# agordon/fastx_toolkit

Measured on AMD Instinct MI355X. Metric: Mreads/s (150 bp) quality-trim+filter, higher is better.
Workload: dtype u8

## Files before the change

fastx_toolkit_amd/csrc/fxg_kernels.h:

```cpp
#pragma once
#include "fxg_device.h"
#include "fxg_clip_instances.h"

#define FXG_INVALID_TUPLE 0xFFFFFFFFu

#define FXG_NTALLY 16
struct FxgLds {
    u32 slot_bytes, so_ksrc, so_kidx, so_ktab;
    u32 off_scratch, off_tally, off_bm_g, off_bm_l, off_bases, off_ptab, total;
    u32 has_tab;
};
__host__ __device__ inline u32 fxg_r16(u32 x) { return (x + 15u) & ~15u; }
__host__ __device__ inline FxgLds fxg_lds_layout(u32 T, u32 stride, u32 bitmaps, u32 stage_stride, u32 nslots = 2, bool no_tab = false, u32 ptab_bytes = 0u)
{
    FxgLds l;
    l.so_ksrc = fxg_r16((T + 1) * 4);
    l.so_kidx = l.so_ksrc + fxg_r16(T * 4);
    l.so_ktab = l.so_kidx + fxg_r16(T * 2);
    l.has_tab = (stage_stride || no_tab) ? 0u : 1u;
    l.slot_bytes = l.so_ktab + (l.has_tab ? fxg_r16(((T * stride + 15) / 16 + 1) * 2) : 0u);
    u32 o = nslots * l.slot_bytes;
    l.off_scratch = o; o += fxg_r16(48 * 4);
    l.off_tally = o;   o += FXG_NTALLY * 8;
    const u32 words = (T * stride + 31) / 32 + 2;
    l.off_bm_g = o;    o += bitmaps ? fxg_r16(words * 4) * (bitmaps == 4u ? 4u : 1u) : 0;
    l.off_bm_l = bitmaps == 1u ? l.off_bm_g : o;    o += bitmaps == 2u ? fxg_r16(words * 4) : 0;
    l.off_bases = o;   o += stage_stride ? fxg_r16(T * stage_stride + 16) : 0;
    l.off_ptab = o;    o += fxg_r16(ptab_bytes);
    l.total = o;
    return l;
}

FXG_HD u32 fxg_bitmap_count(const FxgKArgs &a, bool use_q, bool clip) { return !use_q ? 0u : (clip && a.tq == a.fq) ? 1u : 2u; }

#ifdef FXG_HOST_EMULATION
FXG_HD int fxg_wave_max(int n) { return n; }
#else
__device__ __forceinline__ int fxg_wave_max(int n)
{
    int v = n;
#pragma unroll
    for (int d = 1; d < 64; d <<= 1) { const int o = __shfl_xor(v, d, 64); v = o > v ? o : v; }
    return __builtin_amdgcn_readfirstlane(v);
}
#endif

FXG_HD void fxg_clip_finish(const FxgKArgs &a, int len, int qs, int ts, int mism, int sz, int matches, int bq, int first_n,
                            u32 *out_len, u32 *keep, u32 *reason, u32 *clipped, u32 *adapter_only)
{
    int i = -1;
    if (sz != 0 && !(a.clip_min_adapter_len > 0 && sz < a.clip_min_adapter_len)) {
        if (bq == len - 1 && mism == 0) i = qs;
        else if (sz > 5 && ts == 0 && matches * 100 >= 75 * sz) i = qs;
        else if (sz > 11 && matches * 100 >= 80 * sz) i = qs;
        else if (len >= 2 && bq >= len - 2 && sz <= 5 && matches >= 3) i = qs;
    }
    int cur = len;
    u32 k = 1, why = FXG_R_KEPT, cl = 0, ao = 0;
    if (i > 0) { i += a.clip_keep_delta; if (i < cur) cur = i; cl = 1; }
    if (i == 0) {
        ao = 1;
        if (!(a.clip_flags & FXG_CLIP_ADAPTER_ONLY)) { k = 0; why = FXG_R_CLIP_ADAPTER_ONLY; }
    } else if ((u32)cur < a.clip_min_len) { k = 0; why = FXG_R_CLIP_TOO_SHORT; }
    else if (i == -1 && (a.clip_flags & FXG_CLIP_DISCARD_NON_CLIPPED)) { k = 0; why = FXG_R_CLIP_NO_ADAPTER; }
    else if (i > 0 && (a.clip_flags & FXG_CLIP_DISCARD_CLIPPED)) { k = 0; why = FXG_R_CLIP_ADAPTER_FOUND; }
    else if (!(a.clip_flags & FXG_CLIP_KEEP_N) && first_n < cur) { k = 0; why = FXG_R_CLIP_N; }
    else if (a.clip_flags & FXG_CLIP_ADAPTER_ONLY) { k = 0; why = FXG_R_CLIP_K_MODE; }
    *out_len = (u32)cur; *keep = k; *reason = why; *clipped = cl; *adapter_only = ao;
}

template <int AMAX>
FXG_HD void fxg_clip_read(const FxgKArgs &a, const uint8_t *rd, int len, int rows,
                          u32 *out_len, u32 *keep, u32 *reason, u32 *clipped, u32 *adapter_only, const bool UR = false)
{
    float S[AMAX];
    u32 W0[AMAX], W1[AMAX];
    const int A = a.alen;
#pragma unroll
    for (int t = 0; t < AMAX; ++t) {
        S[t] = (t <= 3) ? 0.0f : -5.0f * (float)(t - 3);
        W0[t] = FXG_INVALID_TUPLE; W1[t] = 0u;
    }
    float best = -1000000.0f;
    u32 bw0 = FXG_INVALID_TUPLE, bw1 = 0u, bq = 0u;
    int first_n = len;
    const int rows_u = UR ? rows : fxg_wave_max(rows);
#pragma unroll 1
    for (int q = 0; q < rows_u; ++q) {
        if (q >= rows) continue;
        const u32 c = rd[q];
        const bool qn = (c == (u32)'N');
        first_n = (qn && first_n == len && q < len) ? q : first_n;
        float dS = 0.0f, uS = 0.0f;
        u32 dW0 = FXG_INVALID_TUPLE, dW1 = 0u, uW0 = FXG_INVALID_TUPLE, uW1 = 0u;
#pragma unroll
        for (int t = 0; t < AMAX; ++t) {
            const u32 tc = (u32)(uint8_t)a.adapter[t];
            const bool tn = (tc == (u32)'N');
            const bool eq = (c == tc);
            const bool neutral = qn || tn;
            const float pair = neutral ? ((qn && tn) ? 0.0f : 0.1f) : (eq ? 1.0f : -1.0f);
            const float ul = dS + pair;
            const float up = uS + -5.0f;
            float left = S[t] + -5.0f;
            if (t > 3) left = (t - 3 > q) ? -100000.0f : left;
            const bool g1 = up > ul;
            float sc = g1 ? up : ul;
            u32 w0 = g1 ? uW0 : dW0, w1 = g1 ? uW1 : dW1;
            const bool g2 = left > sc;
            sc = g2 ? left : sc;
            w0 = g2 ? W0[t] : w0; w1 = g2 ? W1[t] : w1;
            const bool diag = !(g1 || g2);
            const bool fresh = (w0 == FXG_INVALID_TUPLE);
            w0 = fresh ? (((u32)q << 16) | ((u32)t << 8)) : w0;
            w1 = fresh ? 0u : w1;
            w1 += 0x10000u + ((diag && !neutral && eq) ? 1u : 0u);
            w0 += (diag && !neutral && !eq) ? 1u : 0u;
            dS = S[t]; dW0 = W0[t]; dW1 = W1[t];
            S[t] = sc; W0[t] = w0; W1[t] = w1;
            uS = sc; uW0 = w0; uW1 = w1;
            const bool gb = (sc > best) && (t < A);
            best = gb ? sc : best; bw0 = gb ? w0 : bw0; bw1 = gb ? w1 : bw1; bq = gb ? (u32)q : bq;
        }
    }
    fxg_clip_finish(a, len, (int)(bw0 >> 16), (int)((bw0 >> 8) & 0xFFu), (int)(bw0 & 0xFFu), (int)(bw1 >> 16), (int)(bw1 & 0xFFFFu),
                    (int)bq, first_n, out_len, keep, reason, clipped, adapter_only);
}

#define FXG_PK_MAT1  1u
#define FXG_PK_SZ1   (1u << 5)
#define FXG_PK_DIA1  (1u << 14)

template <int AMAX> struct FxgClip2 {
    static constexpr int SPAN = AMAX + (AMAX + 1) / 5;
    static constexpr int C = SPAN / 2 > 0 ? SPAN / 2 : 1;
    static constexpr int WIN = 3 * C;
};

#define FXG_PTAB_LUT_BYTES 512u
#define FXG_PTAB_ROW_BYTES 64u
__host__ __device__ constexpr bool fxg_clip_uses_ptab(int amax) { return amax < 0; }
FXG_HD u32 fxg_ptab_rows(const char *adapter, int alen)
{
    u32 r = 2u;
    for (int t = 0; t < alen; ++t) {
        bool seen = adapter[t] == 'N';
        for (int u = 0; u < t; ++u) seen = seen || (adapter[u] == adapter[t]);
        r += seen ? 0u : 1u;
    }
    return r;
}
FXG_HD u32 fxg_ptab_stride(u32 cols) { const u32 s = (cols * 4u + 15u) & ~15u; return cols <= 16u ? FXG_PTAB_ROW_BYTES : (((s >> 4) & 1u) ? s : s + 16u); }
FXG_HD u32 fxg_ptab_bytes(u32 rows, u32 stride) { return FXG_PTAB_LUT_BYTES + 2u * rows * stride; }
#define FXG_PTAB_MAX_ROWS_K 8u

FXG_HD void fxg_ptab_row_map(const char *adapter, int alen, uint8_t (&row)[256])
{
    for (int b = 0; b < 256; ++b) row[b] = 0u;
    row[0] = 0x80u;
    u32 next = 2u;
    for (int t = 0; t < alen; ++t) {
        const u32 c = (u32)(uint8_t)adapter[t];
        if (c == (u32)'N' || row[c] != 0u) continue;
        row[c] = (uint8_t)(0x80u | next++);
    }
    row[(u32)'N'] = 0x80u | 1u;
}

FXG_HD void fxg_clip_ptab_build(const FxgKArgs &a, uint8_t *ptab, u32 tid, u32 nthreads)
{
    uint16_t *lut = reinterpret_cast<uint16_t *>(ptab);
    const int COLS = (int)a.clip_ptab_cols, A = a.alen < COLS ? a.alen : COLS;
    const u32 R = a.clip_ptab_rows, ST = a.clip_ptab_stride;
    for (u32 b = tid; b < 256u; b += nthreads) {
        const u32 e = a.clip_ptab_row[b], row = e & 0x7Fu;
        lut[b] = (uint16_t)(FXG_PTAB_LUT_BYTES + row * ST);
        if (e & 0x80u) {
            float *pv = reinterpret_cast<float *>(ptab + FXG_PTAB_LUT_BYTES + row * ST);
            u32 *sv = reinterpret_cast<u32 *>(ptab + FXG_PTAB_LUT_BYTES + (R + row) * ST);
            for (int t = 0; t < COLS; ++t) {
                const u32 tc = t < A ? (u32)(uint8_t)a.adapter[t] : 0u;
                const bool eq = tc == b, qn = b == (u32)'N', tn = tc == (u32)'N';
                pv[t] = tn ? (qn ? 0.0f : 0.1f) : (qn ? 0.1f : (eq ? 1.0f : -1.0f));
                sv[t] = (tn || qn) ? 0u : a.clip_ptab_dia1 + (eq ? 1u : 0u);
            }
        }
    }
}

#ifndef FXG_HOST_EMULATION
#define FXG_SCHED_FENCE() __builtin_amdgcn_sched_barrier(0)
#else
#define FXG_SCHED_FENCE() ((void)0)
#endif

FXG_HD float fxg_minus5() { return -5.0f; }

template <int AMAX, bool STEPS>
FXG_HD void fxg_ptab_fetch(const uint8_t *ptab, u32 off, u32 step_off, u32 (&pr)[16], u32 (&st)[16])
{
    const u32x4 *p = reinterpret_cast<const u32x4 *>(ptab + off);
#pragma unroll
    for (int k = 0; k < (AMAX + 3) / 4; ++k) { const u32x4 v = p[k]; pr[4 * k] = v.x; pr[4 * k + 1] = v.y; pr[4 * k + 2] = v.z; pr[4 * k + 3] = v.w; }
    if constexpr (STEPS) {
        const u32x4 *g = reinterpret_cast<const u32x4 *>(ptab + off + step_off);
#pragma unroll
        for (int k = 0; k < (AMAX + 3) / 4; ++k) { const u32x4 v = g[k]; st[4 * k] = v.x; st[4 * k + 1] = v.y; st[4 * k + 2] = v.z; st[4 * k + 3] = v.w; }
    }
}

template <int AMAX, bool EARLY, bool STEPS = false>
FXG_HD float fxg_clip_row_score_t(int A, int q, float (&S)[AMAX], float (&Sm)[AMAX], u32 (&pr)[16], u32 (&st)[16], const uint8_t *ptab, u32 o_next, u32 step_off)
{
    constexpr int AMIN = AMAX <= 4 ? 1 : (AMAX <= 8 ? 5 : AMAX);
    float ul[AMAX];
#pragma unroll
    for (int t = 0; t < AMAX; ++t) ul[t] = (t ? S[t - 1] : 0.0f) + __builtin_bit_cast(float, pr[t]);
    FXG_SCHED_FENCE();
    fxg_ptab_fetch<AMAX, STEPS>(ptab, o_next, step_off, pr, st);
    FXG_SCHED_FENCE();
    const float m5 = fxg_minus5();
    float uSm = -5.0f, rowmax = -1000000.0f;
#pragma unroll
    for (int t = 0; t < AMAX; ++t) {
        float left = Sm[t];
        if (EARLY && t > 3) left = (t - 3 > q) ? -100000.0f : left;
        const float sc = fmaxf(fmaxf(ul[t], uSm), left);
        const float scm = sc + m5;
        S[t] = sc; Sm[t] = scm; uSm = scm;
        if (t < AMIN) rowmax = fmaxf(rowmax, sc);
        else rowmax = (t < A) ? fmaxf(rowmax, sc) : rowmax;
    }
    return rowmax;
}

template <int AMAX, bool EARLY, bool TRACK>
FXG_HD void fxg_clip_row_packed_t(int A, int q, u32 vstart, float (&S)[AMAX], float (&Sm)[AMAX], u32 (&W)[AMAX], float &best, u32 &bw, u32 &bq,
                                  u32 (&pr)[16], u32 (&st)[16], const uint8_t *ptab, u32 o_next, u32 step_off)
{
    const float best_in = best;
    float ul[AMAX];
    u32 wd[AMAX];
#pragma unroll
    for (int t = 0; t < AMAX; ++t) {
        ul[t] = (t ? S[t - 1] : 0.0f) + __builtin_bit_cast(float, pr[t]);
        wd[t] = (t ? W[t - 1] : 0u) + st[t];
    }
    FXG_SCHED_FENCE();
    fxg_ptab_fetch<AMAX, true>(ptab, o_next, step_off, pr, st);
    FXG_SCHED_FENCE();
    const float m5 = fxg_minus5();
    float uSm = -5.0f;
    u32 uW = 0u;
#pragma unroll
    for (int t = 0; t < AMAX; ++t) {
        const float up = uSm;
        float left = Sm[t];
        if (EARLY && t > 3) left = (t - 3 > q) ? -100000.0f : left;
        const float sc = fmaxf(fmaxf(ul[t], up), left);
        const bool isd = (sc == ul[t]), isu = (sc == up);
        u32 w;
        if (t == 0) {
            const u32 src = (isd || isu) ? 0u : W[0];
            const u32 step = isd ? wd[0] : 0u;
            w = (src == 0u) ? ((vstart << 24) + FXG_PK_SZ1 + step) : (src + step);
        } else {
            w = isu ? uW : W[t];
            w = isd ? wd[t] : w;
        }
        const u32 wp = w + FXG_PK_SZ1;
        const float scm = sc + m5;
        S[t] = sc; Sm[t] = scm; W[t] = wp;
        uSm = scm; uW = wp;
        constexpr int AMIN = AMAX <= 4 ? 1 : (AMAX <= 8 ? 5 : (AMAX <= 16 ? AMAX : AMAX - 3));
        if (!TRACK) continue;
        if (t < AMIN) {
            const bool gb = sc > best;
            bw = gb ? w : bw;
            best = fmaxf(best, sc);
        } else {
            const bool gb = (sc > best) && (t < A);
            best = gb ? sc : best; bw = gb ? w : bw;
        }
    }
    if (TRACK) bq = (best > best_in) ? (u32)q : bq;
}

FXG_HD int fxg_gl_last_dword(u64 total, u64 off)
{
    const u64 left = total > off ? (total - off) >> 2 : 0;
    return left == 0 ? 0 : (left - 1 > (u64)0x7FFFFFFF ? 0x7FFFFFFF : (int)(left - 1));
}

FXG_HD u32 fxg_ld32(const uint8_t *row, int i, int imax)
{
    const int k = i < imax ? i : imax;
#ifdef FXG_HOST_EMULATION
    u32 w; memcpy(&w, row + 4 * (size_t)k, 4); return w;
#else
    return reinterpret_cast<const u32 *>(row)[k];
#endif
}

FXG_HD int fxg_clip_first_n(const uint8_t *rd, int len, int len_u, u32 stride, int first_n)
{
    if ((stride & 3u) == 0u) {
#pragma unroll 1
        for (int k = (len_u + 3) / 4 - 1; k >= 0; --k) {
#ifdef FXG_HOST_EMULATION
            u32 w; memcpy(&w, rd + 4 * k, 4);
#else
            const u32 w = reinterpret_cast<const u32 *>(rd)[k];
#endif
            const u32 v = w ^ 0x4E4E4E4Eu;
            const u32 z = (v - 0x01010101u) & ~v & 0x80808080u;
            const int pos = 4 * k + (int)((u32)__builtin_ctz(z | 0x80000000u) >> 3);
            first_n = (z != 0u && pos < len) ? pos : first_n;
        }
    } else {
#pragma unroll 1
        for (int k = len_u - 1; k >= 0; --k) first_n = (k < len && rd[k] == (uint8_t)'N') ? k : first_n;
    }
    return first_n;
}

template <int AMAX, bool GL = false>
FXG_HD int fxg_clip_two_pass(const FxgKArgs &a, const uint8_t *rd, int len, int rows, float &best, u32 &bw, u32 &bq, int &first_n, const bool UR = false, const uint8_t *ptab = nullptr)
{
    constexpr int C = FxgClip2<AMAX>::C;
    float S[AMAX], Sm[AMAX], P0[AMAX], P1[AMAX], P2[AMAX], CB[AMAX];
    const int A = a.alen;
#pragma unroll
    for (int t = 0; t < AMAX; ++t) { S[t] = (t <= 3) ? 0.0f : -5.0f * (float)(t - 3); Sm[t] = S[t] + -5.0f; P0[t] = P1[t] = P2[t] = CB[t] = S[t]; }
    const int early_rows = (A - 4 < rows) ? (A - 4 > 0 ? A - 4 : 0) : rows;
    const int rows_u = UR ? rows : fxg_wave_max(rows > 0 ? rows : 0);
    if (rows_u <= 0) return 0;
    float b1 = -1000000.0f;
    int q = 0, r0 = 0, bq1 = 0;
    u32 cn = 0u, gw0 = 0u, gw1 = 0u;
    int gmax = 0;
    u32 pr[16] = {}, st[16] = {}, on = 0u;
    const u32 step_off = a.clip_ptab_rows * a.clip_ptab_stride;
    const uint16_t *lut = reinterpret_cast<const uint16_t *>(ptab);
    if constexpr (GL) {
        gmax = fxg_gl_last_dword(a.clip_total, (u64)(rd - a.clip_src));
        gw0 = fxg_ld32(rd, 0, gmax); gw1 = fxg_ld32(rd, 1, gmax);
        on = lut[(gw0 >> 8) & 0xFFu];
        fxg_ptab_fetch<AMAX, false>(ptab, lut[gw0 & 0xFFu], step_off, pr, st);
    } else {
        const u32 o0 = lut[rd[0]];
        on = lut[rd[1]]; cn = rd[2];
        fxg_ptab_fetch<AMAX, false>(ptab, o0, step_off, pr, st);
    }
#define FXG_CLIP_CHUNK(EARLY, Psave, Pwin)                                                                                   \
    {                                                                                                                        \
        _Pragma("unroll") for (int t = 0; t < AMAX; ++t) Psave[t] = S[t];                                                    \
        const int q0 = q, qend = q + C < rows_u ? q + C : rows_u;                                                            \
        bool upd = false;                                                                                                    \
        _Pragma("unroll 1") for (; q < qend; ++q) {                                                                          \
            float rm;                                                                                                        \
            if constexpr (GL) {                   \
                const u32 ca = ((((q + 2) >> 2) == (q >> 2) ? gw0 : gw1) >> ((u32)((q + 2) & 3) << 3)) & 0xFFu;             \
                const u32 on2 = lut[ca];                                                                                     \
                if ((q & 3) == 3) { gw0 = gw1; gw1 = fxg_ld32(rd, (q >> 2) + 2, gmax); }                                     \
                if (!UR && q >= rows) continue;                                                                              \
                rm = fxg_clip_row_score_t<AMAX, EARLY>(A, q, S, Sm, pr, st, ptab, on, step_off);                             \
                on = on2;                                                                                                    \
            } else {                                                                                                         \
                if (!UR && q >= rows) continue;           \
                const u32 on2 = lut[cn];                                                                                     \
                cn = rd[q + 3];                                                                                              \
                rm = fxg_clip_row_score_t<AMAX, EARLY>(A, q, S, Sm, pr, st, ptab, on, step_off);                             \
                on = on2;                                                                                                    \
            }                                                                                                                \
            const bool g = rm > b1;                                                                                          \
            b1 = g ? rm : b1; bq1 = g ? q : bq1; upd = upd || g;                                                             \
        }                                                                                                                    \
        if (upd) {                                                                                                           \
            _Pragma("unroll") for (int t = 0; t < AMAX; ++t) CB[t] = Pwin[t];                                                \
            r0 = q0 - 2 * C > 0 ? q0 - 2 * C : 0;                                                                            \
        }                                                                                                                    \
    }
    static_assert(2 * C >= AMAX - 4, "early rows must end inside the first two chunks");
    FXG_CLIP_CHUNK(true, P0, P1)
    if (q < rows_u) FXG_CLIP_CHUNK(true, P1, P2)
    while (q < rows_u) {
        FXG_CLIP_CHUNK(false, P2, P0)
        if (q >= rows_u) break;
        FXG_CLIP_CHUNK(false, P0, P1)
        if (q >= rows_u) break;
        FXG_CLIP_CHUNK(false, P1, P2)
    }
#undef FXG_CLIP_CHUNK
    if (rows <= 0) return 0;
    if (FXG_DBG(a, 32u)) { best = b1; bq = (u32)bq1; bw = 0u; return 0; }
    u32 W[AMAX];
#pragma unroll
    for (int t = 0; t < AMAX; ++t) { S[t] = CB[t]; Sm[t] = CB[t] + -5.0f; W[t] = ((u32)(t + 1) << 19) + FXG_PK_SZ1; }
    q = r0;
    constexpr int SPAN = FxgClip2<AMAX>::SPAN;
    const int rs = bq1 - SPAN + 1 > r0 ? bq1 - SPAN + 1 : r0;
    const int qlast = rows - 1;
#define FXG_RD_AHEAD(i) rd[GL && (i) > qlast ? qlast : (i)]
    {
        const u32 o0 = lut[rd[q]];
        on = lut[FXG_RD_AHEAD(q + 1)]; cn = FXG_RD_AHEAD(q + 2);
        fxg_ptab_fetch<AMAX, true>(ptab, o0, step_off, pr, st);
    }
    const int n0 = rs - r0, n0u = fxg_wave_max(n0);
#pragma unroll 1
    for (int i = 0; i < n0u; ++i) {
        if (i >= n0) continue;
        const u32 on2 = lut[cn];
        cn = FXG_RD_AHEAD(q + 3);
        (void)fxg_clip_row_score_t<AMAX, true, true>(A, q, S, Sm, pr, st, ptab, on, step_off);
        on = on2; ++q;
    }
    const int win = bq1 - rs, n1 = win < early_rows ? win : early_rows, n2 = win - n1;
    const int n1u = fxg_wave_max(n1), n2u = fxg_wave_max(n2);
#pragma unroll 1
    for (int i = 0; i < n1u; ++i) {
        if (i >= n1) continue;
        const u32 on2 = lut[cn];
        cn = FXG_RD_AHEAD(q + 3);
        fxg_clip_row_packed_t<AMAX, true, false>(A, q, (u32)(q - rs), S, Sm, W, best, bw, bq, pr, st, ptab, on, step_off);
        on = on2; ++q;
    }
#pragma unroll 1
    for (int i = 0; i < n2u; ++i) {
        if (i >= n2) continue;
        const u32 on2 = lut[cn];
        cn = FXG_RD_AHEAD(q + 3);
        fxg_clip_row_packed_t<AMAX, false, false>(A, q, (u32)(q - rs), S, Sm, W, best, bw, bq, pr, st, ptab, on, step_off);
        on = on2; ++q;
    }
    fxg_clip_row_packed_t<AMAX, true, true>(A, bq1, (u32)(bq1 - rs), S, Sm, W, best, bw, bq, pr, st, ptab, on, step_off);
#undef FXG_RD_AHEAD
    if (!(a.clip_flags & FXG_CLIP_KEEP_N)) first_n = fxg_clip_first_n(rd, len, UR ? len : fxg_wave_max(len), a.clip_stride, first_n);
    return rs;
}

#define FXG_K_MAT1 1u
#define FXG_K_DIA1 (1u << 7)
#define FXG_K_SZ1  (1u << 14)
#define FXG_K_START(v) ((u32)(v) << 23)
__host__ __device__ constexpr int fxg_clip_k_amin(int amax) { return amax <= 16 ? 1 : fxg_clip_bucket_below(amax) + 1; }
static_assert(fxg_clip_k_amin(16) == 1 && fxg_clip_k_amin(20) == 17 && fxg_clip_k_amin(24) == 21 && fxg_clip_k_amin(64) == 61 && fxg_clip_k_amin(72) == 65 &&
              fxg_clip_k_amin(88) == 81 && fxg_clip_k_amin(100) == 89, "a bucket's smallest adapter is the next smaller bucket + 1");
template <int AMAX> struct FxgClipK { static constexpr bool SM = AMAX <= 24; static constexpr int NSM = SM ? AMAX : 1; };

template <int AMAX, bool EARLY, bool TRACK>
FXG_HD void fxg_clip_row_kt(const FxgKArgs &a, int A, u32 c, int q, u32 vstart, float (&S)[AMAX], float (&Sm)[FxgClipK<AMAX>::NSM], u32 (&W)[AMAX],
                            float &best, u32 &bw, u32 &bq, const uint8_t *ptab)
{
    constexpr bool SM = FxgClipK<AMAX>::SM;
    constexpr int AMIN = fxg_clip_k_amin(AMAX);
    const u32 po = reinterpret_cast<const uint16_t *>(ptab)[c & 0xFFu];
    const u32x4 *pp = reinterpret_cast<const u32x4 *>(ptab + po), *sp = reinterpret_cast<const u32x4 *>(ptab + po + a.clip_ptab_rows * a.clip_ptab_stride);
    const float best_in = best, m5 = fxg_minus5();
    float uSm = -5.0f;
    u32 uW = 0u;
    u32x4 cp = pp[0], cs = sp[0];
    float ul = 0.0f + __builtin_bit_cast(float, cp.x);
    u32 wd = cs.x;
#pragma unroll
    for (int kb = 0; kb < AMAX; kb += 4) {
        u32x4 np = cp, ns = cs;
        if (kb + 4 < AMAX) { np = pp[kb / 4 + 1]; ns = sp[kb / 4 + 1]; }
#pragma unroll
        for (int j = 0; j < 4; ++j) {
            const int t = kb + j;
            if (t >= AMAX) break;
            float ul_next = 0.0f;
            u32 wd_next = 0u;
            if (t + 1 < AMAX) {
                const u32 pv = j == 0 ? cp.y : j == 1 ? cp.z : j == 2 ? cp.w : np.x;
                const u32 sv = j == 0 ? cs.y : j == 1 ? cs.z : j == 2 ? cs.w : ns.x;
                ul_next = S[t] + __builtin_bit_cast(float, pv);
                wd_next = W[t] + sv;
            }
            float left = SM ? Sm[SM ? t : 0] : S[t] + m5;
            if (EARLY && t > 3) left = (t - 3 > q) ? -100000.0f : left;
            const float sc = fmaxf(fmaxf(ul, uSm), left);
            const bool isd = (sc == ul), isu = (sc == uSm);
            u32 w;
            if (t == 0) {
                const u32 fresh = FXG_K_START(vstart) + FXG_K_SZ1 + (isd ? wd : 0u);
                w = (isd || isu) ? fresh : W[0];
            } else {
                w = isu ? uW : W[t];
                w = isd ? wd : w;
            }
            const u32 wp = w + FXG_K_SZ1;
            const float scm = sc + m5;
            S[t] = sc; W[t] = wp;
            if (SM) Sm[SM ? t : 0] = scm;
            uSm = scm; uW = wp; ul = ul_next; wd = wd_next;
            if (!TRACK) continue;
            if (t < AMIN) {
                const bool gb = sc > best;
                bw = gb ? w : bw;
                best = fmaxf(best, sc);
            } else {
                const bool gb = (sc > best) && (t < A);
                best = gb ? sc : best; bw = gb ? w : bw;
            }
        }
        cp = np; cs = ns;
    }
    if (TRACK) bq = (best > best_in) ? (u32)q : bq;
}

template <int AMAX, bool EARLY, bool TRACK>
FXG_HD void fxg_clip_row_k(const FxgKArgs &a, int A, u32 c, int q, u32 vstart, float (&S)[AMAX], float (&Sm)[FxgClipK<AMAX>::NSM], u32 (&W)[AMAX],
                           float &best, u32 &bw, u32 &bq, const uint8_t *ptab)
{
    fxg_clip_row_kt<AMAX, EARLY, TRACK>(a, A, c, q, vstart, S, Sm, W, best, bw, bq, ptab);
}

template <int AMAX, bool EARLY>
FXG_HD float fxg_clip_row_score_k(const FxgKArgs &a, int A, u32 c, int q, float (&S)[AMAX], float (&Sm)[AMAX], const uint8_t *ptab)
{
    constexpr bool SM = AMAX <= 48;
    constexpr int AMIN = fxg_clip_k_amin(AMAX);
    const u32 po = reinterpret_cast<const uint16_t *>(ptab)[c & 0xFFu];
    const u32x4 *pp = reinterpret_cast<const u32x4 *>(ptab + po);
    const float m5 = fxg_minus5();
    float uSm = -5.0f, rowmax = -1000000.0f;
    u32x4 cp = pp[0];
    float ul = 0.0f + __builtin_bit_cast(float, cp.x);
#pragma unroll
    for (int kb = 0; kb < AMAX; kb += 4) {
        u32x4 np = cp;
        if (kb + 4 < AMAX) np = pp[kb / 4 + 1];
#pragma unroll
        for (int j = 0; j < 4; ++j) {
            const int t = kb + j;
            if (t >= AMAX) break;
            float ul_next = 0.0f;
            if (t + 1 < AMAX) ul_next = S[t] + __builtin_bit_cast(float, j == 0 ? cp.y : j == 1 ? cp.z : j == 2 ? cp.w : np.x);
            float left = SM ? Sm[SM ? t : 0] : S[t] + m5;
            if (EARLY && t > 3) left = (t - 3 > q) ? -100000.0f : left;
            const float sc = fmaxf(fmaxf(ul, uSm), left);
            const float scm = sc + m5;
            S[t] = sc;
            if (SM) Sm[SM ? t : 0] = scm;
            uSm = scm; ul = ul_next;
            if (t < AMIN) rowmax = fmaxf(rowmax, sc);
            else rowmax = (t < A) ? fmaxf(rowmax, sc) : rowmax;
        }
        cp = np;
    }
    return rowmax;
}

template <int AMAX>
FXG_HD void fxg_clip_rows_k(const FxgKArgs &a, const uint8_t *rd, int len, int rows, float &best, u32 &bw, u32 &bq, int &first_n, const bool UR = false, const uint8_t *ptab = nullptr)
{
    float S[AMAX], Sm[FxgClipK<AMAX>::NSM];
    u32 W[AMAX];
    const int A = a.alen;
#pragma unroll
    for (int t = 0; t < AMAX; ++t) {
        S[t] = (t <= 3) ? 0.0f : -5.0f * (float)(t - 3);
        if (FxgClipK<AMAX>::SM) Sm[FxgClipK<AMAX>::SM ? t : 0] = S[t] + -5.0f;
        W[t] = FXG_K_START(256 + t + 1) + FXG_K_SZ1;
    }
    const int early_rows = (A - 4 < rows) ? (A - 4 > 0 ? A - 4 : 0) : rows;
    const int early_u = UR ? early_rows : fxg_wave_max(early_rows), rows_u = UR ? rows : fxg_wave_max(rows > 0 ? rows : 0);
    if (rows_u <= 0) return;
    int q = 0;
    u32 cn = rd[0];
#pragma unroll 1
    for (; q < early_u; ++q) {
        const u32 c = cn;
        cn = rd[q + 1];
        if (!UR && q >= rows) continue;
        first_n = (c == (u32)'N' && first_n == len && q < len) ? q : first_n;
        fxg_clip_row_k<AMAX, true, true>(a, A, c, q, (u32)q, S, Sm, W, best, bw, bq, ptab);
    }
#pragma unroll 1
    for (; q < rows_u; ++q) {
        const u32 c = cn;
        cn = rd[q + 1];
        if (!UR && q >= rows) continue;
        first_n = (c == (u32)'N' && first_n == len && q < len) ? q : first_n;
        fxg_clip_row_k<AMAX, false, true>(a, A, c, q, (u32)q, S, Sm, W, best, bw, bq, ptab);
    }
}

template <int AMAX, bool GL = false>
FXG_HD int fxg_clip_two_pass_k(const FxgKArgs &a, const uint8_t *rd, int len, int rows, float *ck, u32 cks, float &best, u32 &bw, u32 &bq, int &first_n, const bool UR = false,
                               const uint8_t *ptab = nullptr)
{
    float S[AMAX], Sm[AMAX];
    const int A = a.alen, K = (int)a.clip_ck_rows;
    const int early_rows = (A - 4 < rows) ? (A - 4 > 0 ? A - 4 : 0) : rows;
    const int early_u = UR ? early_rows : fxg_wave_max(early_rows), rows_u = UR ? rows : fxg_wave_max(rows > 0 ? rows : 0);
    if (rows_u <= 0) return 0;
#pragma unroll
    for (int t = 0; t < AMAX; ++t) { S[t] = (t <= 3) ? 0.0f : -5.0f * (float)(t - 3); Sm[t] = S[t] + -5.0f; }
    float b1 = -1000000.0f;
    int bq1 = 0, next_ck = K, q = 0;
    float *slot = ck;
    u32 cn = 0u, gw0 = 0u, gw1 = 0u;
    int gmax = 0;
    if constexpr (GL) {
        gmax = fxg_gl_last_dword(a.clip_total, (u64)(rd - a.clip_src));
        gw0 = fxg_ld32(rd, 0, gmax); gw1 = fxg_ld32(rd, 1, gmax);
    } else cn = rd[0];
#define FXG_CK_ROW(EARLY)                                                                                                    \
    {                                                                                                                        \
        const bool mine = UR || q < rows;                                                                                    \
        if (q == next_ck) {                                                                                                  \
            if (mine) { _Pragma("unroll") for (int t = 0; t < AMAX; ++t) slot[(size_t)t * cks] = S[t]; }                     \
            slot += (size_t)AMAX * cks; next_ck += K;                                                                        \
        }                                                                                                                    \
        u32 c;                                                                                                               \
        if constexpr (GL) {                                                                                                  \
            c = (gw0 >> ((u32)(q & 3) << 3)) & 0xFFu;                                                                        \
            if ((q & 3) == 3) { gw0 = gw1; gw1 = fxg_ld32(rd, (q >> 2) + 2, gmax); }                                         \
        } else { c = cn; cn = rd[q + 1]; }                                                                                   \
        if (mine) {                                                                                                          \
            const float rm = fxg_clip_row_score_k<AMAX, EARLY>(a, A, c, q, S, Sm, ptab);                                     \
            const bool g = rm > b1;                                                                                          \
            b1 = g ? rm : b1; bq1 = g ? q : bq1;                                                                             \
        }                                                                                                                    \
    }
#pragma unroll 1
    for (; q < early_u; ++q) FXG_CK_ROW(true)
#pragma unroll 1
    for (; q < rows_u; ++q) FXG_CK_ROW(false)
#undef FXG_CK_ROW
    if (rows <= 0) return 0;
    const int span = A + (A + 1) / 5;
    const int r0 = bq1 - span + 1 > 0 ? bq1 - span + 1 : 0;
    const int j0 = r0 / K;
    q = j0 * K;
    {
        const float *from = ck + (size_t)(j0 > 0 ? j0 - 1 : 0) * AMAX * cks;
#pragma unroll
        for (int t = 0; t < AMAX; ++t) {
            const float border = (t <= 3) ? 0.0f : -5.0f * (float)(t - 3);
            S[t] = j0 > 0 ? from[(size_t)t * cks] : border;
            Sm[t] = S[t] + -5.0f;
        }
    }
    {
        const int n0 = r0 - q, n0u = fxg_wave_max(n0);
#pragma unroll 1
        for (int i = 0; i < n0u; ++i) {
            if (i >= n0) continue;
            (void)fxg_clip_row_score_k<AMAX, true>(a, A, (u32)rd[q], q, S, Sm, ptab);
            ++q;
        }
    }
    u32 W[AMAX];
#pragma unroll
    for (int t = 0; t < AMAX; ++t) W[t] = FXG_K_START(256 + t + 1) + FXG_K_SZ1;
    float (&Sk)[FxgClipK<AMAX>::NSM] = reinterpret_cast<float (&)[FxgClipK<AMAX>::NSM]>(Sm);
    const int win = bq1 - r0, n1 = win < early_rows ? win : early_rows, n2 = win - n1;
    const int n1u = fxg_wave_max(n1), n2u = fxg_wave_max(n2);
#pragma unroll 1
    for (int i = 0; i < n1u; ++i) {
        if (i >= n1) continue;
        fxg_clip_row_k<AMAX, true, false>(a, A, (u32)rd[q], q, (u32)(q - r0), S, Sk, W, best, bw, bq, ptab);
        ++q;
    }
#pragma unroll 1
    for (int i = 0; i < n2u; ++i) {
        if (i >= n2) continue;
        fxg_clip_row_k<AMAX, false, false>(a, A, (u32)rd[q], q, (u32)(q - r0), S, Sk, W, best, bw, bq, ptab);
        ++q;
    }
    fxg_clip_row_k<AMAX, true, true>(a, A, (u32)rd[bq1], bq1, (u32)(bq1 - r0), S, Sk, W, best, bw, bq, ptab);
    if (!(a.clip_flags & FXG_CLIP_KEEP_N)) {
        first_n = fxg_clip_first_n(rd, len, UR ? len : fxg_wave_max(len), a.clip_stride, first_n);
    }
    return r0;
}

template <int AMAX, bool KFORM, bool GL = false>
FXG_HD void fxg_clip_read_packed(const FxgKArgs &a, const uint8_t *rd, int len, int rows,
                                 u32 *out_len, u32 *keep, u32 *reason, u32 *clipped, u32 *adapter_only, float *ck = nullptr, u32 cks = 0u, const bool UR = false,
                                 const uint8_t *ptab = nullptr)
{
    float best = -1000000.0f;
    u32 bw = FXG_INVALID_TUPLE, bq = 0u;
    int first_n = len, qbase = 0;
    if constexpr (!KFORM) qbase = fxg_clip_two_pass<AMAX, GL>(a, rd, len, rows, best, bw, bq, first_n, UR, ptab);
    if constexpr (KFORM) {
        int r0 = 0;
        if (ck) r0 = fxg_clip_two_pass_k<AMAX, GL>(a, rd, len, rows, ck, cks, best, bw, bq, first_n, UR, ptab);
        else fxg_clip_rows_k<AMAX>(a, rd, len, rows, best, bw, bq, first_n, UR, ptab);
        const int v = (int)(bw >> 23), matches = (int)(bw & 127u), diag = (int)((bw >> 7) & 127u);
        fxg_clip_finish(a, len, v < 256 ? r0 + v : 0, v < 256 ? 0 : v - 256, diag - matches, (int)((bw >> 14) & 511u), matches,
                        (int)bq, first_n, out_len, keep, reason, clipped, adapter_only);
        return;
    }
    const int matches = (int)(bw & 31u), diag = (int)((bw >> 14) & 31u);
    fxg_clip_finish(a, len, qbase + (int)(bw >> 24), (int)((bw >> 19) & 31u), diag - matches, (int)((bw >> 5) & 511u), matches,
                    (int)bq, first_n, out_len, keep, reason, clipped, adapter_only);
}

struct FxgCounts {
    u64 in, kept, bases, too_short, adapter_only, no_adapter, adapter_found, has_n, qtrim, qfilter, ftrim, k_mode, artifact;
};
#define FXG_RES_ADAPTER_ONLY_BIT 22

FXG_HD void fxg_count_res(u32 w, FxgCounts &c)
{
    const u32 keep = (w >> 16) & 1u, why = (w >> 17) & 0xFu;
    c.in++;
    c.kept += keep;
    c.bases += keep ? (w & 0xFFFFu) : 0u;
    c.adapter_only += (w >> FXG_RES_ADAPTER_ONLY_BIT) & 1u;
    c.too_short += (why == FXG_R_CLIP_TOO_SHORT);
    c.no_adapter += (why == FXG_R_CLIP_NO_ADAPTER);
    c.adapter_found += (why == FXG_R_CLIP_ADAPTER_FOUND);
// ... 521 lines not shown
```

Measured before the change: 12880.

## Drop chunk checkpoints and restart second clip pass from span-bounded row

The first adapter-scoring pass no longer saves per-chunk snapshots of the DP row (P0/P1/P2/CB arrays). It becomes two plain row loops (early rows, then the rest). The second traceback pass now starts directly at the row where the best alignment could begin (best row minus SPAN plus one), with a cleared -1e6 state, instead of replaying rows from a checkpoint. This removes the snapshot copies, the replay rows and several AMAX-sized register arrays, which should cut VGPR pressure. It relies on the alignment length being bounded by SPAN, so results could differ if that assumption fails near the boundary.

```diff
diff --git a/fastx_toolkit_amd/csrc/fxg_kernels.h b/fastx_toolkit_amd/csrc/fxg_kernels.h
--- a/fastx_toolkit_amd/csrc/fxg_kernels.h
+++ b/fastx_toolkit_amd/csrc/fxg_kernels.h
@@ -133,8 +133,6 @@
 
 template <int AMAX> struct FxgClip2 {
     static constexpr int SPAN = AMAX + (AMAX + 1) / 5;
-    static constexpr int C = SPAN / 2 > 0 ? SPAN / 2 : 1;
-    static constexpr int WIN = 3 * C;
 };
 
 #define FXG_PTAB_LUT_BYTES 512u
@@ -209,7 +207,7 @@
     }
 }
 
-template <int AMAX, bool EARLY, bool STEPS = false>
+template <int AMAX, bool EARLY>
 FXG_HD float fxg_clip_row_score_t(int A, int q, float (&S)[AMAX], float (&Sm)[AMAX], u32 (&pr)[16], u32 (&st)[16], const uint8_t *ptab, u32 o_next, u32 step_off)
 {
     constexpr int AMIN = AMAX <= 4 ? 1 : (AMAX <= 8 ? 5 : AMAX);
@@ -217,7 +215,7 @@
 #pragma unroll
     for (int t = 0; t < AMAX; ++t) ul[t] = (t ? S[t - 1] : 0.0f) + __builtin_bit_cast(float, pr[t]);
     FXG_SCHED_FENCE();
-    fxg_ptab_fetch<AMAX, STEPS>(ptab, o_next, step_off, pr, st);
+    fxg_ptab_fetch<AMAX, false>(ptab, o_next, step_off, pr, st);
     FXG_SCHED_FENCE();
     const float m5 = fxg_minus5();
     float uSm = -5.0f, rowmax = -1000000.0f;
@@ -327,16 +325,16 @@
 template <int AMAX, bool GL = false>
 FXG_HD int fxg_clip_two_pass(const FxgKArgs &a, const uint8_t *rd, int len, int rows, float &best, u32 &bw, u32 &bq, int &first_n, const bool UR = false, const uint8_t *ptab = nullptr)
 {
-    constexpr int C = FxgClip2<AMAX>::C;
-    float S[AMAX], Sm[AMAX], P0[AMAX], P1[AMAX], P2[AMAX], CB[AMAX];
+    constexpr int SPAN = FxgClip2<AMAX>::SPAN;
+    float S[AMAX], Sm[AMAX];
     const int A = a.alen;
 #pragma unroll
-    for (int t = 0; t < AMAX; ++t) { S[t] = (t <= 3) ? 0.0f : -5.0f * (float)(t - 3); Sm[t] = S[t] + -5.0f; P0[t] = P1[t] = P2[t] = CB[t] = S[t]; }
+    for (int t = 0; t < AMAX; ++t) { S[t] = (t <= 3) ? 0.0f : -5.0f * (float)(t - 3); Sm[t] = S[t] + -5.0f; }
     const int early_rows = (A - 4 < rows) ? (A - 4 > 0 ? A - 4 : 0) : rows;
     const int rows_u = UR ? rows : fxg_wave_max(rows > 0 ? rows : 0);
     if (rows_u <= 0) return 0;
     float b1 = -1000000.0f;
-    int q = 0, r0 = 0, bq1 = 0;
+    int q = 0, bq1 = 0;
     u32 cn = 0u, gw0 = 0u, gw1 = 0u;
     int gmax = 0;
     u32 pr[16] = {}, st[16] = {}, on = 0u;
@@ -352,69 +350,46 @@
         on = lut[rd[1]]; cn = rd[2];
         fxg_ptab_fetch<AMAX, false>(ptab, o0, step_off, pr, st);
     }
-#define FXG_CLIP_CHUNK(EARLY, Psave, Pwin)                                                                                   \
-    {                                                                                                                        \
-        _Pragma("unroll") for (int t = 0; t < AMAX; ++t) Psave[t] = S[t];                                                    \
-        const int q0 = q, qend = q + C < rows_u ? q + C : rows_u;                                                            \
-        bool upd = false;                                                                                                    \
-        _Pragma("unroll 1") for (; q < qend; ++q) {                                                                          \
-            float rm;                                                                                                        \
-            if constexpr (GL) {                   \
-                const u32 ca = ((((q + 2) >> 2) == (q >> 2) ? gw0 : gw1) >> ((u32)((q + 2) & 3) << 3)) & 0xFFu;             \
-                const u32 on2 = lut[ca];                                                                                     \
-                if ((q & 3) == 3) { gw0 = gw1; gw1 = fxg_ld32(rd, (q >> 2) + 2, gmax); }                                     \
-                if (!UR && q >= rows) continue;                                                                              \
-                rm = fxg_clip_row_score_t<AMAX, EARLY>(A, q, S, Sm, pr, st, ptab, on, step_off);                             \
-                on = on2;                                                                                                    \
-            } else {                                                                                                         \
-                if (!UR && q >= rows) continue;           \
-                const u32 on2 = lut[cn];                                                                                     \
-                cn = rd[q + 3];                                                                                              \
-                rm = fxg_clip_row_score_t<AMAX, EARLY>(A, q, S, Sm, pr, st, ptab, on, step_off);                             \
-                on = on2;                                                                                                    \
-            }                                                                                                                \
-            const bool g = rm > b1;                                                                                          \
-            b1 = g ? rm : b1; bq1 = g ? q : bq1; upd = upd || g;                                                             \
+#define FXG_CLIP_ROWS(EARLY, QEND)                                                                                           \
+    _Pragma("unroll 1") for (; q < (QEND); ++q) {                                                                            \
+        float rm;                                                                                                            \
+        if constexpr (GL) {                       \
+            const u32 ca = ((((q + 2) >> 2) == (q >> 2) ? gw0 : gw1) >> ((u32)((q + 2) & 3) << 3)) & 0xFFu;                 \
+            const u32 on2 = lut[ca];                                                                                         \
+            if ((q & 3) == 3) { gw0 = gw1; gw1 = fxg_ld32(rd, (q >> 2) + 2, gmax); }                                         \
+            if (!UR && q >= rows) continue;                                                                                  \
+            rm = fxg_clip_row_score_t<AMAX, EARLY>(A, q, S, Sm, pr, st, ptab, on, step_off);                                 \
+            on = on2;                                                                                                        \
+        } else {                                                                                                             \
+            if (!UR && q >= rows) continue;               \
+            const u32 on2 = lut[cn];                                                                                         \
+            cn = rd[q + 3];                                                                                                  \
+            rm = fxg_clip_row_score_t<AMAX, EARLY>(A, q, S, Sm, pr, st, ptab, on, step_off);                                 \
+            on = on2;                                                                                                        \
         }                                                                                                                    \
-        if (upd) {                                                                                                           \
-            _Pragma("unroll") for (int t = 0; t < AMAX; ++t) CB[t] = Pwin[t];                                                \
-            r0 = q0 - 2 * C > 0 ? q0 - 2 * C : 0;                                                                            \
-        }                                                                                                                    \
-    }
-    static_assert(2 * C >= AMAX - 4, "early rows must end inside the first two chunks");
-    FXG_CLIP_CHUNK(true, P0, P1)
-    if (q < rows_u) FXG_CLIP_CHUNK(true, P1, P2)
-    while (q < rows_u) {
-        FXG_CLIP_CHUNK(false, P2, P0)
-        if (q >= rows_u) break;
-        FXG_CLIP_CHUNK(false, P0, P1)
-        if (q >= rows_u) break;
-        FXG_CLIP_CHUNK(false, P1, P2)
-    }
-#undef FXG_CLIP_CHUNK
+        const bool g = rm > b1;                                                                                              \
+        b1 = g ? rm : b1; bq1 = g ? q : bq1;                                                                                 \
+    }
+    const int early_u = (A - 4 < rows_u) ? (A - 4 > 0 ? A - 4 : 0) : rows_u;
+    FXG_CLIP_ROWS(true, early_u)
+    FXG_CLIP_ROWS(false, rows_u)
+#undef FXG_CLIP_ROWS
     if (rows <= 0) return 0;
     if (FXG_DBG(a, 32u)) { best = b1; bq = (u32)bq1; bw = 0u; return 0; }
+    const int rs = bq1 - SPAN + 1 > 0 ? bq1 - SPAN + 1 : 0;
     u32 W[AMAX];
 #pragma unroll
-    for (int t = 0; t < AMAX; ++t) { S[t] = CB[t]; Sm[t] = CB[t] + -5.0f; W[t] = ((u32)(t + 1) << 19) + FXG_PK_SZ1; }
-    q = r0;
-    constexpr int SPAN = FxgClip2<AMAX>::SPAN;
-    const int rs = bq1 - SPAN + 1 > r0 ? bq1 - SPAN + 1 : r0;
+    for (int t = 0; t < AMAX; ++t) {
+        const float s0 = (t <= 3) ? 0.0f : -5.0f * (float)(t - 3);
+        S[t] = rs > 0 ? -1000000.0f : s0; Sm[t] = S[t] + -5.0f; W[t] = ((u32)(t + 1) << 19) + FXG_PK_SZ1;
+    }
+    q = rs;
     const int qlast = rows - 1;
 #define FXG_RD_AHEAD(i) rd[GL && (i) > qlast ? qlast : (i)]
     {
         const u32 o0 = lut[rd[q]];
         on = lut[FXG_RD_AHEAD(q + 1)]; cn = FXG_RD_AHEAD(q + 2);
         fxg_ptab_fetch<AMAX, true>(ptab, o0, step_off, pr, st);
-    }
-    const int n0 = rs - r0, n0u = fxg_wave_max(n0);
-#pragma unroll 1
-    for (int i = 0; i < n0u; ++i) {
-        if (i >= n0) continue;
-        const u32 on2 = lut[cn];
-        cn = FXG_RD_AHEAD(q + 3);
-        (void)fxg_clip_row_score_t<AMAX, true, true>(A, q, S, Sm, pr, st, ptab, on, step_off);
-        on = on2; ++q;
     }
     const int win = bq1 - rs, n1 = win < early_rows ? win : early_rows, n2 = win - n1;
     const int n1u = fxg_wave_max(n1), n2u = fxg_wave_max(n2);
```

Result: no change. 12920, median of 4 (+0.3%).
